# apache/yunikorn-k8shim

Measured on AMD Instinct MI355X. Metric: pod×node predicate evals/sec + decisions/sec, 50k nodes × 1M pods, higher is better.
Workload: dtype int64; 1 GPU; configs[2]: 50k nodes x 1M pods, NodeResourcesFit + TaintToleration + NodeAffinity; nodes_per_gpu=50000, total_nodes=50000, pods=1000000, templates=2000, pod_classes=2061, signature_planes=327, unique_requests=False, spread=False, gang_size=0, parallelism=single GPU

## Files before the change

yunikorn-k8shim_amd/csrc/engine/engine.hip:

```cpp
#include "../../../include/ykpred.h"

#include <hip/hip_runtime.h>
#include <dlfcn.h>
#include <rccl/rccl.h>

#include <algorithm>
#include <chrono>
#include <cstdio>
#include <cstdlib>
#include <cstring>
#include <mutex>
#include <string>
#include <unordered_map>
#include <vector>

#include "kernels.hip.h"

using ykk::i64;
using ykk::u64;

namespace {

thread_local std::string g_create_error;

// ... 259 lines not shown
  int rows_total = 0, rows_a = 0, row_capacity = 0;
  DevBuf d_pod_row;
  bool bands_enabled = true;
  int band_steps = 0;
  int band_steps_now = 128;
  int round_batched = -1;
  int round_node_assume = 1;
  int round_prof = 0;
  int fail_after = 0;
  int sig_wpl = 0;
  int combine_slices = 1;
  int decide_groups_from = 16384;
  int early_counts = 1;
  int max_lds_bytes = 64 * 1024;
  int num_cus = 256;
  int n_bands = 0, n_band_steps = 0, n_classes_a = 0, n_fix_rows = 0;
  std::vector<int32_t> h_class_slot_a;
  DevBuf d_band_tab, d_class_rows_a, d_class_list_a, d_class_slot_a, d_fix_row, d_fix_slot, d_chunk_zone;
  DevBuf d_class_list_b;
  int n_classes_b = 0;
  std::vector<int32_t> h_ch_zone;
  std::vector<uint8_t> h_row_stale;
  std::vector<int32_t> h_class_sig, h_class_pin, h_class_first, h_class_live;
  std::vector<std::vector<int32_t>> h_class_chunks;
  std::vector<int32_t> h_members, h_ch_class, h_ch_begin, h_ch_len, h_ch_first;
  int patch_chunks = 0;
  bool rank_valid = false;
  uint64_t specs_version = 1, ranked_specs_version = 0, ranked_nodes_epoch = 0;
  unsigned ranked_pre = 0, ranked_filt = 0;
  bool ranked_has_first = false;
  DevBuf d_round;
  DevBuf d_fx_off, d_fx_cls, d_fx_cnt, d_fx_occ, d_sp_sig_of;
  uint64_t fx_version = 0;
  bool fx_contrib = false, fx_ports = false;
  std::vector<int32_t> h_fx_off;
// ... 203 lines not shown
      long rows = 0;
      for (int c = 0; c < C; ++c)
        if (class_size[(size_t)c] >= need) rows += class_size[(size_t)c];
      return rows;
    };
    const long best = coverage(s_min);
    S = 128;
    while (S > s_min && (double)coverage(S) < 0.5 * (double)best) S /= 2;
  }
  while (S > 4 && (long)S * win / row_b >= (1L << 21)) S -= 4;
  e->band_steps_now = S;
  const int piece_min = piece_min_of(S);
  e->h_class_slot_a.assign((size_t)C, -1);
  e->h_pod_row.assign((size_t)P, -1);
  std::vector<ykk::BandEntry> band_tab;
  std::vector<int32_t> class_list_a, fix_row, fix_slot;
  int n_steps = 0, n_bands = 0, rows_a = 0;
  const bool geometry_ok = e->bands_enabled && e->N > 0 && (size_t)2 * KC * (size_t)row_b <= (size_t)std::min(ykk::kBandMaxLds, e->max_lds_bytes);
  if (geometry_ok) {
    long rows_needed = 0;
    for (int c = 0; c < C; ++c)
      if (class_size[(size_t)c] >= 2 * piece_min) {
        e->h_class_slot_a[(size_t)c] = (int32_t)class_list_a.size();
        class_list_a.push_back(c);
        rows_needed += class_size[(size_t)c];
      }
    if (rows_needed < (long)S * win / row_b / 4) {
      class_list_a.clear();
      std::fill(e->h_class_slot_a.begin(), e->h_class_slot_a.end(), -1);
    }
  }
// ... 87 lines not shown
      rows_a = (int)r_hi;
      if (band_steps_now < S) break;
    }
    if (ci < class_list_a.size()) ok = false;
    if (!ok) {
      class_list_a.clear();
      std::fill(e->h_class_slot_a.begin(), e->h_class_slot_a.end(), -1);
      std::fill(e->h_pod_row.begin(), e->h_pod_row.end(), -1);
      band_tab.clear();
      n_steps = n_bands = rows_a = 0;
    } else {
      n_bands = band;
      std::vector<int32_t> row_slot((size_t)rows_a, -1);
      for (int c : class_list_a)
        for (int i = class_off[(size_t)c]; i < class_off[(size_t)c + 1]; ++i) row_slot[(size_t)e->h_pod_row[(size_t)members[(size_t)i]]] = e->h_class_slot_a[(size_t)c];
      for (long s1 = 1; s1 <= n_steps; ++s1) {
        const long r = (s1 * win - 1) / row_b;
        if (r * row_b + row_b > s1 * win && r < rows_a && row_slot[(size_t)r] >= 0) {
          fix_row.push_back((int32_t)r);
          fix_slot.push_back(row_slot[(size_t)r]);
        }
      }
    }
  }
  int next_row = rows_a;
  e->h_class_sweep.assign((size_t)C, 0);
  e->sweep_ready = false;
  e->sweep_runs = 0;
  e->run_ranges = 0;
  e->walk2_chunks = -1;
  e->index_rows_needed = e->index_rows;
  for (int b = 0; b < ykk::kMaxIdxRows; ++b) e->sweep_rows[b] = 0;
  {
    std::vector<int32_t> order_b;
    for (int c = 0; c < C; ++c)
      if (e->h_class_slot_a[(size_t)c] < 0) order_b.push_back(c);
// ... 95 lines not shown
      if (kx != ky) return kx < ky;
      if (kx == 2) {
        if (cand_big[(size_t)x] != cand_big[(size_t)y]) return cand_big[(size_t)x] < cand_big[(size_t)y];
        if (cand_slot[(size_t)x] != cand_slot[(size_t)y]) return cand_slot[(size_t)x] < cand_slot[(size_t)y];
        if (cand_pos[(size_t)x] != cand_pos[(size_t)y]) return cand_pos[(size_t)x] < cand_pos[(size_t)y];
        return x < y;
      }
      if (key(x, 0) != key(y, 0)) return key(x, 0) < key(y, 0);
      return x < y;
    });
    std::vector<int32_t> first_row_of((size_t)C, -1);
    for (int32_t c : order_b) {
      first_row_of[(size_t)c] = next_row;
      for (int i = class_off[(size_t)c]; i < class_off[(size_t)c + 1]; ++i) e->h_pod_row[(size_t)members[(size_t)i]] = next_row++;
    }
    e->n_classes_b = (int)order_b.size();
    TRY(upload(e, e->d_class_list_b, order_b.data(), order_b.size(), st));
    std::vector<ykk::SweepRun> runs;
    e->run_classes = e->run_units = e->run_rows = 0;
    if (runs_possible) {
      std::vector<ykk::RunClass> rcs;
      std::vector<int32_t> starts;
      for (size_t i = 0; i < order_b.size();) {
        const int32_t c = order_b[i];
        if (kind_of(c) != 1) {
          ++i;
          continue;
        }
        size_t j = i;
        long rows_in_run = 0;
// ... 230 lines not shown
            if (sr >= 0)
              for (int k = 0; k < R1; ++k)
                if (e->h_res_rows[(size_t)sr * (size_t)R1 + (size_t)k] > 0 && (e->h_res_rows[(size_t)sr * (size_t)R1 + (size_t)k] >> ykk::kRowBigShift)) { ++t_single_big; break; }
          }
        }
        fprintf(stderr, "fused: %d classes, %d rows, %d combinations; chunk writers keep %ld classes / %ld rows of zone B (%ld single-row: %ld share their affinity signature, %ld with an index row, %ld spread, %ld pinned)\n",
                e->fuse_count, e->fuse_row_count, e->fuse_combos, t_cls, t_rows, t_single, t_single_shared, t_single_big, t_single_spread, t_pinned);
      }
    }
  }
  e->rows_total = next_row;
  e->rows_a = rows_a;
  e->n_bands = n_bands;
  e->n_band_steps = n_steps;
  e->n_classes_a = (int)class_list_a.size();
  e->n_fix_rows = (int)fix_row.size();
  if (e->row_capacity && e->rows_total > e->row_capacity)
    return fail(e, YKPRED_E_INVALID, "the bitmap needs more rows than ykpred_set_row_capacity allows");
  const int cm = e->chunk_members;
  struct Chunk {
    int32_t cls, begin, len, first, first_row;
  };
  std::vector<Chunk> chunks;
  for (int c = 0; c < C; ++c)
    for (int b = class_off[(size_t)c]; b < class_off[(size_t)c + 1]; b += cm)
      chunks.push_back({c, b, std::min(cm, class_off[(size_t)c + 1] - b), b == class_off[(size_t)c] ? 1 : 0, e->h_pod_row[(size_t)members[(size_t)b]]});
  if (e->chunk_sorted)
    std::stable_sort(chunks.begin(), chunks.end(), [](const Chunk& x, const Chunk& y) { return x.first_row < y.first_row; });
  auto &ch_class = e->h_ch_class, &ch_begin = e->h_ch_begin, &ch_len = e->h_ch_len, &ch_first = e->h_ch_first;
  ch_class.clear();
  ch_begin.clear();
// ... 27 lines not shown
  e->h_row_stale.assign((size_t)P, 0);
  e->C = C;
  e->NC = (int)ch_class.size();
  e->patch_chunks = 0;
  TRY(upload(e, e->d_pod_class, pod_class.data(), pod_class.size(), st));
  TRY(upload(e, e->d_class_sig, class_sig.data(), class_sig.size(), st));
  TRY(upload(e, e->d_class_pin, class_pin.data(), class_pin.size(), st));
  TRY(upload(e, e->d_class_first, e->h_class_first.data(), e->h_class_first.size(), st));
  TRY(upload(e, e->d_members, member_rows.data(), member_rows.size(), st));
  TRY(upload(e, e->d_pod_row, e->h_pod_row.data(), e->h_pod_row.size(), st));
  TRY(upload(e, e->d_chunk_zone, e->h_ch_zone.data(), e->h_ch_zone.size(), st));
  TRY(upload(e, e->d_chunk_list_b, chunk_list_b.data(), chunk_list_b.size(), st));
  TRY(upload(e, e->d_band_tab, band_tab.data(), band_tab.size(), st));
  TRY(upload(e, e->d_class_list_a, class_list_a.data(), class_list_a.size(), st));
  TRY(upload(e, e->d_class_slot_a, e->h_class_slot_a.data(), e->h_class_slot_a.size(), st));
  TRY(upload(e, e->d_fix_row, fix_row.data(), fix_row.size(), st));
  TRY(upload(e, e->d_fix_slot, fix_slot.data(), fix_slot.size(), st));
  HIPCHK(e->d_class_rows_a.ensure((size_t)std::max<size_t>(class_list_a.size(), 1) * (size_t)e->row_stride * sizeof(u64)));
  TRY(upload(e, e->d_chunk_class, ch_class.data(), ch_class.size(), st));
  TRY(upload(e, e->d_chunk_begin, ch_begin.data(), ch_begin.size(), st));
  TRY(upload(e, e->d_chunk_len, ch_len.data(), ch_len.size(), st));
  TRY(upload(e, e->d_chunk_first, ch_first.data(), ch_first.size(), st));
  HIPCHK(e->d_class_count.ensure((size_t)std::max(C, 1) * sizeof(int)));
  HIPCHK(e->d_class_best.ensure((size_t)std::max(C, 1) * sizeof(int)));
  HIPCHK(hipStreamSynchronize(st));
  e->classes_dirty = false;
  e->layout_version++;
  e->last_eval_valid = false;
  return YKPRED_OK;
}

int ensure_planes(ykpred_engine* e, hipStream_t st) {
  int rows = 0;
// ... 454 lines not shown
  if (e->comm) (void)rccl()->CommDestroy(e->comm);
  e->comm = nullptr;
  for (DevBuf* b : {&e->d_gathered, &e->d_gathered_map, &e->d_xkey, &e->d_xcand}) b->release();
  for (auto& g : e->graphs) (void)hipGraphExecDestroy(g.second);
  e->graphs.clear();
  for (DevBuf* b : {&e->d_alloc, &e->d_req, &e->d_allowed, &e->d_count, &e->d_nflags, &e->d_taints, &e->d_labels, &e->d_domain, &e->d_selcount, &e->d_ports, &e->d_sig_ports, &e->d_swanted,
                    &e->d_sp_cnt_prev, &e->d_sp_present_prev, &e->d_sp_min_prev, &e->d_sig_changed, &e->d_class_dirty,
                    &e->d_spec_spread, &e->d_sp_coff, &e->d_sp_c, &e->d_sp_aff, &e->d_sp_tol, &e->d_sp_cnt, &e->d_sp_present, &e->d_sp_min,
                    &e->planes_canon, &e->planes_ranked, &e->base_canon, &e->base_ranked, &e->d_rankbuf, &e->d_score, &e->d_key,
                    &e->d_rank, &e->d_perm, &e->d_sreq, &e->d_stol, &e->d_sflags, &e->d_aff_off, &e->d_aff_terms, &e->d_pre_off,
                    &e->d_pre_terms, &e->d_dim_val, &e->d_dim_order, &e->d_dim_chunk_dim, &e->d_dim_chunk_begin, &e->d_dim_chunk_len,
                    &e->d_res_rows, &e->d_big_dim, &e->d_walk_big, &e->d_walk_begin, &e->d_walk_len, &e->d_sfree_c, &e->d_pmask_c,
                    &e->d_sfree_r, &e->d_pmask_r, &e->d_rbits_c, &e->d_sorted, &e->d_sorted_off, &e->d_ent_c, &e->d_agree, &e->d_topo_agree, &e->d_bytes_gather, &e->d_fuse_rec, &e->d_fuse_combo_rec, &e->d_fuse_combo, &e->d_run_ranges, &e->d_no_decide, &e->d_glin_r, &e->d_run_classes, &e->d_run_units, &e->d_sweep_rows, &e->d_sweep_runs, &e->d_sweep_units, &e->d_chunk_list_b0, &e->d_walk2_order, &e->d_walk2_big, &e->d_walk2_begin, &e->d_walk2_len, &e->d_idx_c, &e->d_win_r, &e->d_pfx_r, &e->d_slice_desc, &e->d_slice_general, &e->d_chunk_list_b, &e->d_first_r, &e->d_sig_tol, &e->d_sig_tolflags, &e->d_sig_aff_flags, &e->d_sig_aff_off,
                    &e->d_sig_aff_terms, &e->d_sig_pre_off, &e->d_sig_pre_terms, &e->d_pod_spec, &e->d_pod_pin, &e->d_pod_class,
                    &e->d_class_sig, &e->d_class_pin, &e->d_class_first, &e->d_class_word, &e->d_chunk_class, &e->d_chunk_begin, &e->d_chunk_len, &e->d_chunk_first,
                    &e->d_pod_row, &e->d_band_tab, &e->d_class_rows_a, &e->d_class_list_a, &e->d_class_slot_a, &e->d_fix_row, &e->d_fix_slot, &e->d_chunk_zone,
                    &e->d_members, &e->d_patches, &e->d_rows, &e->d_row_count, &e->d_row_best, &e->d_class_count, &e->d_class_best, &e->d_bitmap, &e->d_counts, &e->d_decisions, &e->d_keys, &e->d_scratch,
                    &e->d_member_key, &e->d_name_rank, &e->d_member_tie, &e->d_class_rows_all, &e->d_gathered_classes, &e->d_class_rows_slot,
                    &e->d_class_sig_ident, &e->d_expand_count, &e->d_layout_hash, &e->d_gathered_pod_class, &e->d_row_pod,
                    &e->d_round, &e->d_fx_off, &e->d_fx_cls, &e->d_fx_cnt, &e->d_fx_occ, &e->d_sp_sig_of, &e->d_class_list_b, &e->d_gathered, &e->d_gathered_map,
                    &e->d_xkey, &e->d_xcand})
    b->release();
  if (e->ev_ready)
    for (auto& ev : e->ev) (void)hipEventDestroy(ev);
  if (e->ev_fork) (void)hipEventDestroy(e->ev_fork);
  if (e->ev_join) (void)hipEventDestroy(e->ev_join);
  if (e->ev_planes) (void)hipEventDestroy(e->ev_planes);
  if (e->ev_counts) (void)hipEventDestroy(e->ev_counts);
  if (e->ev_zero) (void)hipEventDestroy(e->ev_zero);
  if (e->h_round_pinned) (void)hipHostFree(e->h_round_pinned);
  if (e->ev_eval_done) (void)hipEventDestroy(e->ev_eval_done);
// ... 791 lines not shown
                         pr, n_decide, e->row_words, e->d_perm.as<int>(), e->d_rank.as<int>(), pin_on, e->d_class_best.as<int>(), n_decide <= 4096 ? 1 : 0);
    }
    tm.end(sb, "k_decide");
  }
  const bool skip_combine = a->options & YKPRED_EVAL_SKIP_BITMAP;
  const bool dirty_only = a->options & YKPRED_EVAL_DIRTY_CLASSES;
  const int* class_dirty = nullptr;
  if (!skip_combine && dirty_only) {
    HIPCHK(e->d_class_dirty.ensure((size_t)std::max(e->C, 1) * sizeof(int)));
    hipLaunchKernelGGL(ykk::k_mark_dirty_classes, dim3((unsigned)((e->C + ykk::kBlock - 1) / ykk::kBlock)), dim3(ykk::kBlock), 0, st, e->C,
                       e->d_class_sig.as<int>(), e->d_sig_changed.as<int>(), e->d_class_dirty.as<int>(), e->d_class_count.as<int>());
    class_dirty = e->d_class_dirty.as<int>();
  }
  const bool small_chunks = (long)e->NC * e->wave_combine_below > (long)P;
  const bool counts_early = e->early_counts != 0 && !skip_combine && !dirty_only && e->n_classes_a > 0 && e->patch_chunks == 0 && !small_chunks && e->n_classes_b <= 16384;
  bool scattered = false;
  if (!skip_combine && !dirty_only && !counts_early) {
    if (zero_counts_beside) HIPCHK(hipStreamWaitEvent(st, e->ev_zero, 0));
    else HIPCHK(hipMemsetAsync(e->d_class_count.p, 0, (size_t)e->C * sizeof(int), st));
  }
  if (!skip_combine) {
    int tpg = ykk::kBlock;
    while (tpg > ykk::kWave && (tpg / 2) * 2 >= e->row_stride) tpg /= 2;
    const int seg = tpg * ykk::kCombineUnroll * 2;
    const bool listed = !dirty_only && e->patch_chunks == 0;
    const bool short_list = use_sweep && (fuse_on || e->fuse_count == 0);
    const int* chunk_list = listed ? (short_list ? e->d_chunk_list_b0 : e->d_chunk_list_b).as<int>() : nullptr;
    const int n_run = listed ? (short_list ? e->NCB0 : e->NCB) : e->NC;
    dim3 grid((unsigned)std::max(n_run, 1), (unsigned)((e->row_stride + seg - 1) / seg));
    hipStream_t sz = st;
    if (!dirty_only && e->n_classes_a > 0) {
      tm.begin(st);
      const int n_counted_b = counts_early ? e->n_classes_b : 0;
      hipLaunchKernelGGL(ykk::k_class_rows, dim3((unsigned)((e->n_classes_a + n_counted_b + ykk::kWavesPerBlock - 1) / ykk::kWavesPerBlock)), dim3(ykk::kBlock), 0, st,
                         ct, pc, e->d_class_list_a.as<int>(), e->n_classes_a, e->row_words, e->row_stride, pin_on, e->d_class_rows_a.as<u64>(),
                         e->d_class_count.as<int>(), (const int*)nullptr, e->d_class_list_b.as<int>(), n_counted_b);
      tm.end(st, "k_class_rows");
      if (counts_early && want_dec) {
        HIPCHK(hipEventRecord(e->ev_counts, st));
        HIPCHK(hipStreamWaitEvent(sb, e->ev_counts, 0));
        tm.begin(sb);
        hipLaunchKernelGGL(ykk::k_scatter, dim3((unsigned)((P + ykk::kBlock - 1) / ykk::kBlock)), dim3(ykk::kBlock), 0, sb, P,
                           e->d_pod_class.as<int>(), e->d_class_count.as<int>(), e->d_class_best.as<int>(), e->d_key.as<u64>(),
                           want_cnt ? (int*)e->last_counts : nullptr, (int*)e->last_decisions, want_keys ? (i64*)e->last_keys : nullptr);
        tm.end(sb, "k_scatter");
        scattered = true;
      }
      const size_t lds_bytes = (size_t)2 * ykk::kBandClasses * (size_t)e->row_stride * sizeof(u64);
      if (lds_bytes > 64 * 1024)
        HIPCHK(hipFuncSetAttribute((const void*)ykk::k_expand_bands, hipFuncAttributeMaxDynamicSharedMemorySize, (int)lds_bytes));
      tm.begin(st);
      hipLaunchKernelGGL(ykk::k_expand_bands, dim3((unsigned)ykk::kBandGroups), dim3(ykk::kBandBlock), lds_bytes, st, bitmap,
                         e->d_class_rows_a.as<u64>(), e->d_band_tab.as<ykk::BandEntry>(), e->n_bands, e->row_stride);
      if (e->n_fix_rows > 0 && !counts_early)
        hipLaunchKernelGGL(ykk::k_fix_rows, dim3((unsigned)e->n_fix_rows), dim3(ykk::kBlock), 0, st, bitmap, e->d_class_rows_a.as<u64>(),
                           e->d_fix_row.as<int>(), e->d_fix_slot.as<int>(), e->n_fix_rows, e->row_stride);
      tm.end(st, "k_expand_bands");
    }
    if (use_sweep && e->run_classes > 0) {
      ykk::WalkStage rstage{};
      rstage.n = (int)e->h_stage_rows.size();
      for (int k = 0; k < rstage.n; ++k) rstage.row[k] = e->h_stage_rows[(size_t)k];
      const int its = (e->row_stride + ykk::kWave - 1) / ykk::kWave;
      int segs = (its + ykk::kWalkMaxIt - 1) / ykk::kWalkMaxIt, nit = (its + segs - 1) / segs;
      while (nit > 1 && ykk::runs_lds_bytes(rstage.n, nit) > (size_t)e->max_lds_bytes) {
        ++segs;
        nit = (its + segs - 1) / segs;
      }
      const int n_long = segs - (nit * segs - its);
      const size_t lds = ykk::runs_lds_bytes(rstage.n, nit);
      const int per_cu = lds * 2 <= (size_t)e->max_lds_bytes ? 2 : 1;
// ... 66 lines not shown
      auto launch_wide = [&](const ykk::FuseRec* recs, int n, u64* out, int* counts) {
        if (wpl == 5) launch_fused(ykk::k_fused_rows<5, 8>, recs, n, out, counts);
        else if (wpl == 2) launch_fused(ykk::k_fused_rows<2, 8>, recs, n, out, counts);
        else launch_fused(ykk::k_fused_rows<1, 8>, recs, n, out, counts);
      };
      if (e->fuse_combos > 0) {
        launch_wide(e->d_fuse_combo_rec.as<ykk::FuseRec>(), e->fuse_combos, e->d_fuse_combo.as<u64>(), nullptr);
        if (wpl == 5) launch_fused(ykk::k_fused_rows<5, 2>, e->d_fuse_rec.as<ykk::FuseRec>(), e->fuse_count, bitmap, e->d_class_count.as<int>());
        else if (wpl == 2) launch_fused(ykk::k_fused_rows<2, 2>, e->d_fuse_rec.as<ykk::FuseRec>(), e->fuse_count, bitmap, e->d_class_count.as<int>());
        else launch_fused(ykk::k_fused_rows<1, 2>, e->d_fuse_rec.as<ykk::FuseRec>(), e->fuse_count, bitmap, e->d_class_count.as<int>());
      } else {
        launch_wide(e->d_fuse_rec.as<ykk::FuseRec>(), e->fuse_count, bitmap, e->d_class_count.as<int>());
      }
      tm.end(sz, "k_fused_rows");
    }
    tm.begin(sz);
    int walk_nit = 0, walk_segs = 0, walk_long = 0;
    ykk::WalkStage wstage{};
    wstage.n = (int)e->h_stage_rows.size();
    for (int k = 0; k < wstage.n; ++k) wstage.row[k] = e->h_stage_rows[(size_t)k];
    bool slices = small_chunks && e->combine_slices != 0 && pc.n_big > 0 && pc.res != nullptr && !(use_sweep && e->sweep_min_run <= 1 && listed);
    if (slices) {
      const int its = (e->row_stride + ykk::kWave - 1) / ykk::kWave;
      const size_t lds_cap = std::min((size_t)e->max_lds_bytes, (size_t)80 * 1024);
      walk_segs = (its + ykk::kWalkMaxIt - 1) / ykk::kWalkMaxIt;
      walk_nit = (its + walk_segs - 1) / walk_segs;
      while (walk_nit > 1 && ykk::walk_lds_bytes(pc.n_big, wstage.n, walk_nit) > lds_cap) {
        ++walk_segs;
        walk_nit = (its + walk_segs - 1) / walk_segs;
      }
      walk_long = walk_segs - (walk_nit * walk_segs - its);
// ... 27 lines not shown
        }
        return fail(e, YKPRED_E_INVALID, "k_walk_rows: no kernel for " + std::to_string(nit) + " word groups per lane");
      };
      {
        const int n_short = walk_segs - walk_long, nit_last = n_short > 0 ? walk_nit - 1 : walk_nit;
        const int long_plain = n_short > 0 ? walk_long : walk_long - 1, short_plain = n_short > 0 ? n_short - 1 : 0;
        TRY(launch_segments(walk_nit, long_plain, 0, false));
        TRY(launch_segments(walk_nit - 1, short_plain, walk_long * walk_nit * ykk::kWave, false));
        TRY(launch_segments(nit_last, 1, (long_plain * walk_nit + short_plain * (walk_nit - 1)) * ykk::kWave, true));
      }
      tm.end(sz, "k_walk_rows");
      tm.begin(sz);
      hipLaunchKernelGGL(ykk::k_combine_wave, dim3((unsigned)((e->NC + ykk::kWavesPerBlock - 1) / ykk::kWavesPerBlock)), dim3(ykk::kBlock), 0, sz, ct,
                         pc, bitmap, e->row_words, e->row_stride, pin_on, e->d_class_count.as<int>(), e->NC, class_dirty,
                         e->d_slice_desc.as<ykk::SliceDesc>(), e->d_slice_general.as<int>(), (const int*)nullptr);
    } else if (counts_early) {
      const ykk::FixRows fix{e->d_class_rows_a.as<u64>(), e->d_fix_row.as<int>(), e->d_fix_slot.as<int>(), e->n_fix_rows};
      const int blocks = n_run + e->n_fix_rows;
      if (blocks > 0)
        hipLaunchKernelGGL(ykk::k_combine, dim3((unsigned)blocks, grid.y), dim3(ykk::kBlock), (size_t)e->combine_lds_bytes, sz, ct, pc, bitmap, e->row_words,
                           e->row_stride, pin_on, (int*)nullptr, tpg, class_dirty, chunk_list, fix, n_run);
    } else if (n_run == 0) {
    } else if (small_chunks) {
      const dim3 wgrid((unsigned)((std::max(n_run, 1) + ykk::kWavesPerBlock - 1) / ykk::kWavesPerBlock));
      hipLaunchKernelGGL(ykk::k_combine_wave, wgrid, dim3(ykk::kBlock), 0, sz, ct, pc, bitmap, e->row_words, e->row_stride, pin_on,
                         e->d_class_count.as<int>(), n_run, class_dirty, (const ykk::SliceDesc*)nullptr, (const int*)nullptr, chunk_list);
    } else {
      hipLaunchKernelGGL(ykk::k_combine, grid, dim3(ykk::kBlock), (size_t)e->combine_lds_bytes, sz, ct, pc, bitmap, e->row_words, e->row_stride,
                         pin_on, e->d_class_count.as<int>(), tpg, class_dirty, chunk_list, ykk::FixRows{nullptr, nullptr, nullptr, 0}, n_run);
    }
    tm.end(sz, dirty_only ? "k_combine(dirty classes)" : "k_combine");
  }
  if (want_dec) {
    HIPCHK(hipEventRecord(e->ev_join, sb));
    HIPCHK(hipStreamWaitEvent(st, e->ev_join, 0));
  }
  if ((want_dec || want_cnt) && !scattered) {
    tm.begin(st);
    hipLaunchKernelGGL(ykk::k_scatter, dim3((unsigned)((P + ykk::kBlock - 1) / ykk::kBlock)), dim3(ykk::kBlock), 0, st, P,
                       e->d_pod_class.as<int>(), e->d_class_count.as<int>(), e->d_class_best.as<int>(), e->d_key.as<u64>(),
                       want_cnt ? (int*)e->last_counts : nullptr, want_dec ? (int*)e->last_decisions : nullptr,
                       want_keys ? (i64*)e->last_keys : nullptr);
    tm.end(st, "k_scatter");
  }
  HIPCHK(hipGetLastError());
  return YKPRED_OK;
// ... 1761 lines not shown
    hipLaunchKernelGGL(ykk::k_identity_sigs, dim3((unsigned)((C + ykk::kBlock - 1) / ykk::kBlock)), dim3(ykk::kBlock), 0, st, C, e->d_class_sig_ident.as<int>());
    e->ident_classes = C;
  }
  HIPCHK(e->d_expand_count.ensure((size_t)C * sizeof(int)));
  ykk::ClassTable ct{e->d_class_sig_ident.as<int>(), e->d_class_pin.as<int>(), e->d_chunk_class.as<int>(), e->d_chunk_begin.as<int>(),
                     e->d_chunk_len.as<int>(), e->d_chunk_first.as<int>(), e->d_members.as<int>(), e->d_chunk_zone.as<int>(), 0, nullptr};
  ykk::Planes pl{nullptr, class_rows, nullptr, nullptr, e->row_stride, nullptr, 0, nullptr, 0, nullptr, 0, nullptr, 0, 0, 0, 0, 0, nullptr, nullptr, nullptr, nullptr, nullptr};
  if (e->n_classes_a > 0) {
    HIPCHK(e->d_class_rows_slot.ensure((size_t)e->n_classes_a * (size_t)e->row_stride * sizeof(u64)));
    hipLaunchKernelGGL(ykk::k_pick_class_rows, dim3((unsigned)e->n_classes_a), dim3(ykk::kBlock), 0, st, class_rows, e->d_class_list_a.as<int>(),
                       e->n_classes_a, e->row_stride, e->d_class_rows_slot.as<u64>());
    const size_t lds_bytes = (size_t)2 * ykk::kBandClasses * (size_t)e->row_stride * sizeof(u64);
    if (lds_bytes > 64 * 1024)
      HIPCHK(hipFuncSetAttribute((const void*)ykk::k_expand_bands, hipFuncAttributeMaxDynamicSharedMemorySize, (int)lds_bytes));
    hipLaunchKernelGGL(ykk::k_expand_bands, dim3((unsigned)ykk::kBandGroups), dim3(ykk::kBandBlock), lds_bytes, st, out, e->d_class_rows_slot.as<u64>(),
                       e->d_band_tab.as<ykk::BandEntry>(), e->n_bands, e->row_stride);
    if (e->n_fix_rows > 0)
      hipLaunchKernelGGL(ykk::k_fix_rows, dim3((unsigned)e->n_fix_rows), dim3(ykk::kBlock), 0, st, out, e->d_class_rows_slot.as<u64>(),
                         e->d_fix_row.as<int>(), e->d_fix_slot.as<int>(), e->n_fix_rows, e->row_stride);
  }
  if ((long)e->NC * e->wave_combine_below > (long)P) {
    hipLaunchKernelGGL(ykk::k_combine_wave, dim3((unsigned)((e->NC + ykk::kWavesPerBlock - 1) / ykk::kWavesPerBlock)), dim3(ykk::kBlock), 0, st, ct, pl,
                       out, e->row_stride, e->row_stride, 0, e->d_expand_count.as<int>(), e->NC, (const int*)nullptr, (const ykk::SliceDesc*)nullptr,
                       (const int*)nullptr, (const int*)nullptr);
  } else {
    int tpg = ykk::kBlock;
    while (tpg > ykk::kWave && (tpg / 2) * 2 >= e->row_stride) tpg /= 2;
    const int seg = tpg * ykk::kCombineUnroll * 2;
    dim3 grid((unsigned)e->NC, (unsigned)((e->row_stride + seg - 1) / seg));
    hipLaunchKernelGGL(ykk::k_combine, grid, dim3(ykk::kBlock), (size_t)e->combine_lds_bytes, st, ct, pl, out, e->row_stride, e->row_stride, 0,
                       e->d_expand_count.as<int>(), tpg, (const int*)nullptr, (const int*)nullptr, ykk::FixRows{nullptr, nullptr, nullptr, 0}, e->NC);
  }
  HIPCHK(hipGetLastError());
  return YKPRED_OK;
}
int expand_peer_rows_into(ykpred_engine_t* e, const u64* class_rows, const int* pod_class, u64* out, hipStream_t st) {
  if (e->P == 0) return YKPRED_OK;
  const int n_rows = std::max(std::max(e->rows_total, e->row_capacity), 1);
  if (e->row_pod_version != e->layout_version) {
    HIPCHK(e->d_row_pod.ensure((size_t)n_rows * sizeof(int)));
    HIPCHK(hipMemsetAsync(e->d_row_pod.p, 0xff, (size_t)n_rows * sizeof(int), st));
    hipLaunchKernelGGL(ykk::k_invert_row_map, dim3((unsigned)((e->P + ykk::kBlock - 1) / ykk::kBlock)), dim3(ykk::kBlock), 0, st, e->d_pod_row.as<int>(), e->P,
                       e->d_row_pod.as<int>());
    e->row_pod_version = e->layout_version;
  }
  const int row_groups = (n_rows + ykk::kExpandRows - 1) / ykk::kExpandRows;
// ... 178 lines not shown
```

yunikorn-k8shim_amd/csrc/engine/kernels.hip.h:

```cpp
#pragma once
#include <hip/hip_runtime.h>
#include <stdint.h>

#include <type_traits>

namespace ykk {

typedef unsigned long long u64;
typedef long long i64;

constexpr int kMaxR = 8;
constexpr int kMaxKT = 4;
constexpr int kMaxW = 8;
constexpr int kMaxWTotal = 32;
constexpr int kMaxKD = 8;
constexpr int kMaxKP = 4;

constexpr int kWave = 64;
constexpr int kBlock = 256;
constexpr int kWavesPerBlock = kBlock / kWave;
constexpr int kSigsPerBlock = 16;
constexpr int kSigsPerBlockMany = 64;
constexpr int kManySigs = 4096;
__host__ __device__ inline int sigs_per_block(int D) { return D > kManySigs ? kSigsPerBlockMany : kSigsPerBlock; }
// ... 1058 lines not shown
        pos = lo;
      }
      v &= cr.ipm[i][(size_t)w * 65 + min(pos, 64)];
    }
  return v;
}
__device__ __forceinline__ u64 class_word(const ClassRows& cr, int w) {
  u64 v = ~0ull;
#pragma unroll
  for (int i = 0; i < kMaxClassRows; ++i)
    if (i < cr.n) v &= cr.row[i][w];
  if (cr.ni) v &= class_idx_word(cr, w);
  return v;
}

struct FixRows {
  const u64* class_rows;
  const int* rows;
  const int* slots;
  int n;
};
__device__ __forceinline__ void fix_row(const FixRows& f, int i, u64* __restrict__ out, int row_stride) {
  typedef u64 u64x2 __attribute__((ext_vector_type(2)));
  if (i >= f.n) return;
  const u64* src = f.class_rows + (size_t)f.slots[i] * row_stride;
  u64* dst = out + (size_t)f.rows[i] * row_stride;
  for (int w = threadIdx.x * 2; w < row_stride; w += 2 * kBlock) *(u64x2*)(dst + w) = *(const u64x2*)(src + w);
}
__global__ __launch_bounds__(kBlock) void k_combine(ClassTable ct, Planes pl, u64* __restrict__ bitmap, int row_words, int row_stride,
                                                    int pin_enabled, int* __restrict__ class_count, int tpg,
                                                    const int* __restrict__ class_dirty ,
                                                    const int* __restrict__ chunk_list ,
                                                    FixRows fix ,
                                                    int n_run) {
  constexpr int WPL = 2;
  if ((int)blockIdx.x >= n_run) {
    if (blockIdx.y == 0) fix_row(fix, (int)blockIdx.x - n_run, bitmap, row_stride);
    return;
  }
  const bool all_fail = pin_enabled & 2;
  pin_enabled &= 1;
  const int chunk = chunk_list ? chunk_list[blockIdx.x] : (int)blockIdx.x;
  const int cls = ct.chunk_class[chunk];
  if (class_dirty ? !class_dirty[cls] : chunk_elsewhere(ct, chunk)) return;
  const int begin = ct.chunk_begin[chunk];
  const int len = ct.chunk_len[chunk];
  const int sr = ct.sig[cls * 4 + 0], st = ct.sig[cls * 4 + 1], sa = ct.sig[cls * 4 + 2], ss = ct.sig[cls * 4 + 3];
  const int pin = pin_enabled ? ct.pin[cls] : -1;
  const int lane = threadIdx.x % kWave;
  const int group = threadIdx.x / tpg, groups = kBlock / tpg, t = threadIdx.x % tpg;
  const int seg_base = blockIdx.y * (tpg * kCombineUnroll * WPL);
  const ClassRows cr = class_rows(pl, sr, st, sa, ss);

  u64 v[kCombineUnroll][WPL];
// ... 763 lines not shown
      if (__builtin_amdgcn_readfirstlane(db.x) != run) break;
    }
  }
}

constexpr int kBandGroups = 256;
constexpr int kBandClasses = 4;
constexpr int kBandMaxLds = 150 * 1024;
struct BandEntry {
  int slot[kBandClasses];
  int xb[kBandClasses - 1];
  int sb[kBandClasses - 1];
  int steps, first_step;
  int n, pad;
};

__global__ __launch_bounds__(kBlock) void k_class_rows(ClassTable ct, Planes pl, const int* __restrict__ class_list, int n_list, int row_words,
                                                       int row_stride, int pin_enabled, u64* __restrict__ row_table,
                                                       int* __restrict__ class_count, const int* __restrict__ class_dirty,
                                                       const int* __restrict__ class_list_b, int n_b) {
  typedef u64 u64x2 __attribute__((ext_vector_type(2)));
  const bool all_fail = pin_enabled & 2;
  pin_enabled &= 1;
  const int k = blockIdx.x * kWavesPerBlock + threadIdx.x / kWave;
  if (k >= n_list + n_b) return;
  const bool store = k < n_list;
  const int cls = store ? class_list[k] : class_list_b[k - n_list];
  if (class_dirty && !class_dirty[cls]) return;
  const int lane = threadIdx.x % kWave;
  const int sr = ct.sig[cls * 4 + 0], st = ct.sig[cls * 4 + 1], sa = ct.sig[cls * 4 + 2], ss = ct.sig[cls * 4 + 3];
  const int pin = pin_enabled ? ct.pin[cls] : -1;
  const ClassRows cr = class_rows(pl, sr, st, sa, ss);
  u64* dst = row_table + (size_t)k * row_stride;
  int pc = 0;
  for (int w = 2 * lane; w < row_stride; w += 2 * kWave) {
    u64x2 x = {0, 0};
    if (w < row_words && pin != -2 && !all_fail) {
      x = u64x2{~0ull, ~0ull};
#pragma unroll
      for (int i = 0; i < kMaxClassRows; ++i)
        if (i < cr.n) x &= *(const u64x2*)(cr.row[i] + w);
      if (cr.ni) {
// ... 4 lines not shown
      if (pin >= 0) {
        x.x &= (w == (pin >> 6)) ? (1ull << (pin & 63)) : 0ull;
        x.y &= (w + 1 == (pin >> 6)) ? (1ull << (pin & 63)) : 0ull;
      }
    }
    pc += __popcll(x.x) + __popcll(x.y);
    if (store) *(u64x2*)(dst + w) = x;
  }
#pragma unroll
  for (int off = 32; off > 0; off >>= 1) pc += __shfl_down(pc, off, kWave);
  if (lane == 0) class_count[cls] = pc;
}

constexpr int kBandBlock = kBlock + kWave;
__global__ __launch_bounds__(kBandBlock) void k_expand_bands(u64* __restrict__ out, const u64* __restrict__ class_rows,
                                                             const BandEntry* __restrict__ tab, int n_bands, int row_stride) {
  typedef u64 u64x2 __attribute__((ext_vector_type(2)));
  extern __shared__ u64 band_lds[];
  const int b = blockIdx.x, tid = threadIdx.x;
  const int row_b = row_stride * 8;
  constexpr long kWin = (long)kBandGroups * 4096;
  if (tid >= kBlock) {
    const int lane = tid - kBlock;
    const int pieces = row_stride / 2;
    auto load_rows = [&](int band) {
      const BandEntry be = tab[(size_t)band * kBandGroups + b];
#pragma unroll
      for (int c = 0; c < kBandClasses; ++c) {
        if (c >= be.n && c > 0) break;
        const u64x2* src = (const u64x2*)(class_rows + (size_t)be.slot[c] * row_stride);
        u64x2* dst = (u64x2*)(band_lds + (size_t)((band & 1) * kBandClasses + c) * row_stride);
        for (int i0 = 0; i0 < pieces; i0 += 4 * kWave) {
          u64x2 r[4];
#pragma unroll
          for (int k = 0; k < 4; ++k)
            if (i0 + k * kWave + lane < pieces) r[k] = src[i0 + k * kWave + lane];
#pragma unroll
          for (int k = 0; k < 4; ++k)
            if (i0 + k * kWave + lane < pieces) dst[i0 + k * kWave + lane] = r[k];
        }
      }
    };
    load_rows(0);
    __syncthreads();
    for (int band = 0; band < n_bands; ++band) {
      if (band + 1 < n_bands) load_rows(band + 1);
      __syncthreads();
    }
    return;
  }
  __syncthreads();
  const int p = b * 4096 + tid * 16;
  const unsigned urow_b = (unsigned)row_b;
  const unsigned dcol = (unsigned)(kWin % row_b);
  unsigned ucol = (unsigned)(p % row_b);
  for (int band = 0; band < n_bands; ++band) {
    const BandEntry cur = tab[(size_t)band * kBandGroups + b];
    const int s0 = cur.first_step, s1 = s0 + cur.steps;
    const char* lds = (const char*)(band_lds + (size_t)(band & 1) * kBandClasses * row_stride);
    unsigned kb[kBandClasses - 1];
#pragma unroll
// ... 24 lines not shown
          if (live[u]) *(u64x2*)(win_base + p) = v[u];
          win_base += kWin;
        }
      }
    };
    if (cur.n <= 1)
      run_band(std::integral_constant<int, 1>{});
    else if (cur.n == 2)
      run_band(std::integral_constant<int, 2>{});
    else if (cur.n == 3)
      run_band(std::integral_constant<int, 3>{});
    else
      run_band(std::integral_constant<int, kBandClasses>{});
    __syncthreads();
  }
}
__global__ __launch_bounds__(kBlock) void k_fix_rows(u64* __restrict__ out, const u64* __restrict__ class_rows, const int* __restrict__ rows,
                                                     const int* __restrict__ slots, int n, int row_stride) {
  typedef u64 u64x2 __attribute__((ext_vector_type(2)));
  if ((int)blockIdx.x >= n) return;
  const u64* src = class_rows + (size_t)slots[blockIdx.x] * row_stride;
  u64* dst = out + (size_t)rows[blockIdx.x] * row_stride;
  for (int w = threadIdx.x * 2; w < row_stride; w += 2 * kBlock) *(u64x2*)(dst + w) = *(const u64x2*)(src + w);
}

__global__ __launch_bounds__(kBlock) void k_decide(ClassTable ct, Planes ranked, int n_classes, int row_words, const int* __restrict__ perm,
                                                   const int* __restrict__ rank, int pin_enabled, int* __restrict__ class_best, int eager) {
  int cls = blockIdx.x * kWavesPerBlock + threadIdx.x / kWave;
  if (cls >= n_classes) return;
  if (ct.decide_list) cls = ct.decide_list[cls];
  const int lane = threadIdx.x % kWave;
  const int sr = ct.sig[cls * 4 + 0], st = ct.sig[cls * 4 + 1], sa = ct.sig[cls * 4 + 2], ss = ct.sig[cls * 4 + 3];
  const bool all_fail = pin_enabled & 2;
  const int pin = (pin_enabled & 1) ? ct.pin[cls] : -1;
  int best = -1;
  const ClassRows cr = class_rows(ranked, sr, st, sa, ss);
  if (pin == -2 || all_fail) {
    best = -1;
// ... 1940 lines not shown
```

Before: 42760 billion evals/s.

## Fold boundary-row fixups and B-class rows into band expansion kernel

Removes the separate k_fix_rows launch and the fix-row tail blocks in k_combine. The partial head of each band-boundary row is now copied inside k_expand_bands from the class row table. When the B-class rows fit within the band step count, k_class_rows also stores the B-class rows into the slot table. The band kernel's loader wave then copies them into the bitmap, letting the trailing k_combine launch be skipped. This costs extra row-table memory and puts more copy work on the band loader wave.

Result: slower. 42020 billion evals/s (-1.7%).

```diff
diff --git a/yunikorn-k8shim_amd/csrc/engine/engine.hip b/yunikorn-k8shim_amd/csrc/engine/engine.hip
--- a/yunikorn-k8shim_amd/csrc/engine/engine.hip
+++ b/yunikorn-k8shim_amd/csrc/engine/engine.hip
@@ -297,11 +297,12 @@
   int early_counts = 1;
   int max_lds_bytes = 64 * 1024;
   int num_cus = 256;
-  int n_bands = 0, n_band_steps = 0, n_classes_a = 0, n_fix_rows = 0;
+  int n_bands = 0, n_band_steps = 0, n_classes_a = 0;
   std::vector<int32_t> h_class_slot_a;
-  DevBuf d_band_tab, d_class_rows_a, d_class_list_a, d_class_slot_a, d_fix_row, d_fix_slot, d_chunk_zone;
+  DevBuf d_band_tab, d_class_rows_a, d_class_list_a, d_class_slot_a, d_head_slot, d_ride_slot, d_chunk_zone;
   DevBuf d_class_list_b;
   int n_classes_b = 0;
+  int n_ride_rows = 0, ride_rows_total = 0;
   std::vector<int32_t> h_ch_zone;
   std::vector<uint8_t> h_row_stale;
   std::vector<int32_t> h_class_sig, h_class_pin, h_class_first, h_class_live;
@@ -535,7 +536,7 @@
   e->h_class_slot_a.assign((size_t)C, -1);
   e->h_pod_row.assign((size_t)P, -1);
   std::vector<ykk::BandEntry> band_tab;
-  std::vector<int32_t> class_list_a, fix_row, fix_slot;
+  std::vector<int32_t> class_list_a, head_slot, ride_slot;
   int n_steps = 0, n_bands = 0, rows_a = 0;
   const bool geometry_ok = e->bands_enabled && e->N > 0 && (size_t)2 * KC * (size_t)row_b <= (size_t)std::min(ykk::kBandMaxLds, e->max_lds_bytes);
   if (geometry_ok) {
@@ -653,12 +654,10 @@
       std::vector<int32_t> row_slot((size_t)rows_a, -1);
       for (int c : class_list_a)
         for (int i = class_off[(size_t)c]; i < class_off[(size_t)c + 1]; ++i) row_slot[(size_t)e->h_pod_row[(size_t)members[(size_t)i]]] = e->h_class_slot_a[(size_t)c];
+      head_slot.assign((size_t)n_steps + 1, -1);
       for (long s1 = 1; s1 <= n_steps; ++s1) {
         const long r = (s1 * win - 1) / row_b;
-        if (r * row_b + row_b > s1 * win && r < rows_a && row_slot[(size_t)r] >= 0) {
-          fix_row.push_back((int32_t)r);
-          fix_slot.push_back(row_slot[(size_t)r]);
-        }
+        if (r * row_b + row_b > s1 * win && r < rows_a) head_slot[(size_t)s1] = row_slot[(size_t)r];
       }
     }
   }
@@ -784,6 +783,8 @@
       first_row_of[(size_t)c] = next_row;
       for (int i = class_off[(size_t)c]; i < class_off[(size_t)c + 1]; ++i) e->h_pod_row[(size_t)members[(size_t)i]] = next_row++;
     }
+    if (rows_a > 0 && next_row - rows_a <= n_steps)
+      for (size_t k = 0; k < order_b.size(); ++k) ride_slot.insert(ride_slot.end(), (size_t)class_size[(size_t)order_b[k]], (int32_t)(class_list_a.size() + k));
     e->n_classes_b = (int)order_b.size();
     TRY(upload(e, e->d_class_list_b, order_b.data(), order_b.size(), st));
     std::vector<ykk::SweepRun> runs;
@@ -1044,7 +1045,8 @@
   e->n_bands = n_bands;
   e->n_band_steps = n_steps;
   e->n_classes_a = (int)class_list_a.size();
-  e->n_fix_rows = (int)fix_row.size();
+  e->n_ride_rows = (int)ride_slot.size();
+  e->ride_rows_total = next_row;
   if (e->row_capacity && e->rows_total > e->row_capacity)
     return fail(e, YKPRED_E_INVALID, "the bitmap needs more rows than ykpred_set_row_capacity allows");
   const int cm = e->chunk_members;
@@ -1102,9 +1104,9 @@
   TRY(upload(e, e->d_band_tab, band_tab.data(), band_tab.size(), st));
   TRY(upload(e, e->d_class_list_a, class_list_a.data(), class_list_a.size(), st));
   TRY(upload(e, e->d_class_slot_a, e->h_class_slot_a.data(), e->h_class_slot_a.size(), st));
-  TRY(upload(e, e->d_fix_row, fix_row.data(), fix_row.size(), st));
-  TRY(upload(e, e->d_fix_slot, fix_slot.data(), fix_slot.size(), st));
-  HIPCHK(e->d_class_rows_a.ensure((size_t)std::max<size_t>(class_list_a.size(), 1) * (size_t)e->row_stride * sizeof(u64)));
+  TRY(upload(e, e->d_head_slot, head_slot.data(), head_slot.size(), st));
+  TRY(upload(e, e->d_ride_slot, ride_slot.data(), ride_slot.size(), st));
+  HIPCHK(e->d_class_rows_a.ensure((size_t)std::max<size_t>(class_list_a.size() + (ride_slot.empty() ? 0 : (size_t)e->n_classes_b), 1) * (size_t)e->row_stride * sizeof(u64)));
   TRY(upload(e, e->d_chunk_class, ch_class.data(), ch_class.size(), st));
   TRY(upload(e, e->d_chunk_begin, ch_begin.data(), ch_begin.size(), st));
   TRY(upload(e, e->d_chunk_len, ch_len.data(), ch_len.size(), st));
@@ -1589,7 +1591,7 @@
                     &e->d_sfree_r, &e->d_pmask_r, &e->d_rbits_c, &e->d_sorted, &e->d_sorted_off, &e->d_ent_c, &e->d_agree, &e->d_topo_agree, &e->d_bytes_gather, &e->d_fuse_rec, &e->d_fuse_combo_rec, &e->d_fuse_combo, &e->d_run_ranges, &e->d_no_decide, &e->d_glin_r, &e->d_run_classes, &e->d_run_units, &e->d_sweep_rows, &e->d_sweep_runs, &e->d_sweep_units, &e->d_chunk_list_b0, &e->d_walk2_order, &e->d_walk2_big, &e->d_walk2_begin, &e->d_walk2_len, &e->d_idx_c, &e->d_win_r, &e->d_pfx_r, &e->d_slice_desc, &e->d_slice_general, &e->d_chunk_list_b, &e->d_first_r, &e->d_sig_tol, &e->d_sig_tolflags, &e->d_sig_aff_flags, &e->d_sig_aff_off,
                     &e->d_sig_aff_terms, &e->d_sig_pre_off, &e->d_sig_pre_terms, &e->d_pod_spec, &e->d_pod_pin, &e->d_pod_class,
                     &e->d_class_sig, &e->d_class_pin, &e->d_class_first, &e->d_class_word, &e->d_chunk_class, &e->d_chunk_begin, &e->d_chunk_len, &e->d_chunk_first,
-                    &e->d_pod_row, &e->d_band_tab, &e->d_class_rows_a, &e->d_class_list_a, &e->d_class_slot_a, &e->d_fix_row, &e->d_fix_slot, &e->d_chunk_zone,
+                    &e->d_pod_row, &e->d_band_tab, &e->d_class_rows_a, &e->d_class_list_a, &e->d_class_slot_a, &e->d_head_slot, &e->d_ride_slot, &e->d_chunk_zone,
                     &e->d_members, &e->d_patches, &e->d_rows, &e->d_row_count, &e->d_row_best, &e->d_class_count, &e->d_class_best, &e->d_bitmap, &e->d_counts, &e->d_decisions, &e->d_keys, &e->d_scratch,
                     &e->d_member_key, &e->d_name_rank, &e->d_member_tie, &e->d_class_rows_all, &e->d_gathered_classes, &e->d_class_rows_slot,
                     &e->d_class_sig_ident, &e->d_expand_count, &e->d_layout_hash, &e->d_gathered_pod_class, &e->d_row_pod,
@@ -2411,6 +2413,7 @@
   }
   const bool small_chunks = (long)e->NC * e->wave_combine_below > (long)P;
   const bool counts_early = e->early_counts != 0 && !skip_combine && !dirty_only && e->n_classes_a > 0 && e->patch_chunks == 0 && !small_chunks && e->n_classes_b <= 16384;
+  const bool ride = counts_early && e->n_ride_rows > 0 && e->rows_total == e->ride_rows_total;
   bool scattered = false;
   if (!skip_combine && !dirty_only && !counts_early) {
     if (zero_counts_beside) HIPCHK(hipStreamWaitEvent(st, e->ev_zero, 0));
@@ -2431,7 +2434,7 @@
       const int n_counted_b = counts_early ? e->n_classes_b : 0;
       hipLaunchKernelGGL(ykk::k_class_rows, dim3((unsigned)((e->n_classes_a + n_counted_b + ykk::kWavesPerBlock - 1) / ykk::kWavesPerBlock)), dim3(ykk::kBlock), 0, st,
                          ct, pc, e->d_class_list_a.as<int>(), e->n_classes_a, e->row_words, e->row_stride, pin_on, e->d_class_rows_a.as<u64>(),
-                         e->d_class_count.as<int>(), (const int*)nullptr, e->d_class_list_b.as<int>(), n_counted_b);
+                         e->d_class_count.as<int>(), (const int*)nullptr, e->d_class_list_b.as<int>(), n_counted_b, ride ? 1 : 0);
       tm.end(st, "k_class_rows");
       if (counts_early && want_dec) {
         HIPCHK(hipEventRecord(e->ev_counts, st));
@@ -2448,10 +2451,8 @@
         HIPCHK(hipFuncSetAttribute((const void*)ykk::k_expand_bands, hipFuncAttributeMaxDynamicSharedMemorySize, (int)lds_bytes));
       tm.begin(st);
       hipLaunchKernelGGL(ykk::k_expand_bands, dim3((unsigned)ykk::kBandGroups), dim3(ykk::kBandBlock), lds_bytes, st, bitmap,
-                         e->d_class_rows_a.as<u64>(), e->d_band_tab.as<ykk::BandEntry>(), e->n_bands, e->row_stride);
-      if (e->n_fix_rows > 0 && !counts_early)
-        hipLaunchKernelGGL(ykk::k_fix_rows, dim3((unsigned)e->n_fix_rows), dim3(ykk::kBlock), 0, st, bitmap, e->d_class_rows_a.as<u64>(),
-                           e->d_fix_row.as<int>(), e->d_fix_slot.as<int>(), e->n_fix_rows, e->row_stride);
+                         e->d_class_rows_a.as<u64>(), e->d_band_tab.as<ykk::BandEntry>(), e->n_bands, e->row_stride,
+                         ykk::BandRide{e->d_head_slot.as<int>(), e->d_ride_slot.as<int>(), ride ? e->n_ride_rows : 0, e->rows_a});
       tm.end(st, "k_expand_bands");
     }
     if (use_sweep && e->run_classes > 0) {
@@ -2548,7 +2549,8 @@
       }
       tm.end(sz, "k_fused_rows");
     }
-    tm.begin(sz);
+    const bool tail = !(ride || (counts_early && n_run == 0));
+    if (tail) tm.begin(sz);
     int walk_nit = 0, walk_segs = 0, walk_long = 0;
     ykk::WalkStage wstage{};
     wstage.n = (int)e->h_stage_rows.size();
@@ -2606,12 +2608,11 @@
       hipLaunchKernelGGL(ykk::k_combine_wave, dim3((unsigned)((e->NC + ykk::kWavesPerBlock - 1) / ykk::kWavesPerBlock)), dim3(ykk::kBlock), 0, sz, ct,
                          pc, bitmap, e->row_words, e->row_stride, pin_on, e->d_class_count.as<int>(), e->NC, class_dirty,
                          e->d_slice_desc.as<ykk::SliceDesc>(), e->d_slice_general.as<int>(), (const int*)nullptr);
+    } else if (ride) {
     } else if (counts_early) {
-      const ykk::FixRows fix{e->d_class_rows_a.as<u64>(), e->d_fix_row.as<int>(), e->d_fix_slot.as<int>(), e->n_fix_rows};
-      const int blocks = n_run + e->n_fix_rows;
-      if (blocks > 0)
-        hipLaunchKernelGGL(ykk::k_combine, dim3((unsigned)blocks, grid.y), dim3(ykk::kBlock), (size_t)e->combine_lds_bytes, sz, ct, pc, bitmap, e->row_words,
-                           e->row_stride, pin_on, (int*)nullptr, tpg, class_dirty, chunk_list, fix, n_run);
+      if (n_run > 0)
+        hipLaunchKernelGGL(ykk::k_combine, grid, dim3(ykk::kBlock), (size_t)e->combine_lds_bytes, sz, ct, pc, bitmap, e->row_words, e->row_stride, pin_on,
+                           (int*)nullptr, tpg, class_dirty, chunk_list, n_run);
     } else if (n_run == 0) {
     } else if (small_chunks) {
       const dim3 wgrid((unsigned)((std::max(n_run, 1) + ykk::kWavesPerBlock - 1) / ykk::kWavesPerBlock));
@@ -2619,9 +2620,9 @@
                          e->d_class_count.as<int>(), n_run, class_dirty, (const ykk::SliceDesc*)nullptr, (const int*)nullptr, chunk_list);
     } else {
       hipLaunchKernelGGL(ykk::k_combine, grid, dim3(ykk::kBlock), (size_t)e->combine_lds_bytes, sz, ct, pc, bitmap, e->row_words, e->row_stride,
-                         pin_on, e->d_class_count.as<int>(), tpg, class_dirty, chunk_list, ykk::FixRows{nullptr, nullptr, nullptr, 0}, n_run);
-    }
-    tm.end(sz, dirty_only ? "k_combine(dirty classes)" : "k_combine");
+                         pin_on, e->d_class_count.as<int>(), tpg, class_dirty, chunk_list, n_run);
+    }
+    if (tail) tm.end(sz, dirty_only ? "k_combine(dirty classes)" : "k_combine");
   }
   if (want_dec) {
     HIPCHK(hipEventRecord(e->ev_join, sb));
@@ -4413,10 +4414,7 @@
     if (lds_bytes > 64 * 1024)
       HIPCHK(hipFuncSetAttribute((const void*)ykk::k_expand_bands, hipFuncAttributeMaxDynamicSharedMemorySize, (int)lds_bytes));
     hipLaunchKernelGGL(ykk::k_expand_bands, dim3((unsigned)ykk::kBandGroups), dim3(ykk::kBandBlock), lds_bytes, st, out, e->d_class_rows_slot.as<u64>(),
-                       e->d_band_tab.as<ykk::BandEntry>(), e->n_bands, e->row_stride);
-    if (e->n_fix_rows > 0)
-      hipLaunchKernelGGL(ykk::k_fix_rows, dim3((unsigned)e->n_fix_rows), dim3(ykk::kBlock), 0, st, out, e->d_class_rows_slot.as<u64>(),
-                         e->d_fix_row.as<int>(), e->d_fix_slot.as<int>(), e->n_fix_rows, e->row_stride);
+                       e->d_band_tab.as<ykk::BandEntry>(), e->n_bands, e->row_stride, ykk::BandRide{e->d_head_slot.as<int>(), nullptr, 0, e->rows_a});
   }
   if ((long)e->NC * e->wave_combine_below > (long)P) {
     hipLaunchKernelGGL(ykk::k_combine_wave, dim3((unsigned)((e->NC + ykk::kWavesPerBlock - 1) / ykk::kWavesPerBlock)), dim3(ykk::kBlock), 0, st, ct, pl,
@@ -4428,7 +4426,7 @@
     const int seg = tpg * ykk::kCombineUnroll * 2;
     dim3 grid((unsigned)e->NC, (unsigned)((e->row_stride + seg - 1) / seg));
     hipLaunchKernelGGL(ykk::k_combine, grid, dim3(ykk::kBlock), (size_t)e->combine_lds_bytes, st, ct, pl, out, e->row_stride, e->row_stride, 0,
-                       e->d_expand_count.as<int>(), tpg, (const int*)nullptr, (const int*)nullptr, ykk::FixRows{nullptr, nullptr, nullptr, 0}, e->NC);
+                       e->d_expand_count.as<int>(), tpg, (const int*)nullptr, (const int*)nullptr, e->NC);
   }
   HIPCHK(hipGetLastError());
   return YKPRED_OK;
diff --git a/yunikorn-k8shim_amd/csrc/engine/kernels.hip.h b/yunikorn-k8shim_amd/csrc/engine/kernels.hip.h
--- a/yunikorn-k8shim_amd/csrc/engine/kernels.hip.h
+++ b/yunikorn-k8shim_amd/csrc/engine/kernels.hip.h
@@ -1096,30 +1096,13 @@
   return v;
 }
 
-struct FixRows {
-  const u64* class_rows;
-  const int* rows;
-  const int* slots;
-  int n;
-};
-__device__ __forceinline__ void fix_row(const FixRows& f, int i, u64* __restrict__ out, int row_stride) {
-  typedef u64 u64x2 __attribute__((ext_vector_type(2)));
-  if (i >= f.n) return;
-  const u64* src = f.class_rows + (size_t)f.slots[i] * row_stride;
-  u64* dst = out + (size_t)f.rows[i] * row_stride;
-  for (int w = threadIdx.x * 2; w < row_stride; w += 2 * kBlock) *(u64x2*)(dst + w) = *(const u64x2*)(src + w);
-}
 __global__ __launch_bounds__(kBlock) void k_combine(ClassTable ct, Planes pl, u64* __restrict__ bitmap, int row_words, int row_stride,
                                                     int pin_enabled, int* __restrict__ class_count, int tpg,
                                                     const int* __restrict__ class_dirty ,
                                                     const int* __restrict__ chunk_list ,
-                                                    FixRows fix ,
                                                     int n_run) {
   constexpr int WPL = 2;
-  if ((int)blockIdx.x >= n_run) {
-    if (blockIdx.y == 0) fix_row(fix, (int)blockIdx.x - n_run, bitmap, row_stride);
-    return;
-  }
+  if ((int)blockIdx.x >= n_run) return;
   const bool all_fail = pin_enabled & 2;
   pin_enabled &= 1;
   const int chunk = chunk_list ? chunk_list[blockIdx.x] : (int)blockIdx.x;
@@ -1913,18 +1896,24 @@
   int steps, first_step;
   int n, pad;
 };
+struct BandRide {
+  const int* head_slot;
+  const int* ride_slot;
+  int n_ride, first_row;
+};
+constexpr int kBandPiece = 1024;
 
 __global__ __launch_bounds__(kBlock) void k_class_rows(ClassTable ct, Planes pl, const int* __restrict__ class_list, int n_list, int row_words,
                                                        int row_stride, int pin_enabled, u64* __restrict__ row_table,
                                                        int* __restrict__ class_count, const int* __restrict__ class_dirty,
-                                                       const int* __restrict__ class_list_b, int n_b) {
+                                                       const int* __restrict__ class_list_b, int n_b, int store_b) {
   typedef u64 u64x2 __attribute__((ext_vector_type(2)));
   const bool all_fail = pin_enabled & 2;
   pin_enabled &= 1;
   const int k = blockIdx.x * kWavesPerBlock + threadIdx.x / kWave;
   if (k >= n_list + n_b) return;
-  const bool store = k < n_list;
-  const int cls = store ? class_list[k] : class_list_b[k - n_list];
+  const bool store = k < n_list || store_b;
+  const int cls = k < n_list ? class_list[k] : class_list_b[k - n_list];
   if (class_dirty && !class_dirty[cls]) return;
   const int lane = threadIdx.x % kWave;
   const int sr = ct.sig[cls * 4 + 0], st = ct.sig[cls * 4 + 1], sa = ct.sig[cls * 4 + 2], ss = ct.sig[cls * 4 + 3];
@@ -1959,7 +1948,7 @@
 
 constexpr int kBandBlock = kBlock + kWave;
 __global__ __launch_bounds__(kBandBlock) void k_expand_bands(u64* __restrict__ out, const u64* __restrict__ class_rows,
-                                                             const BandEntry* __restrict__ tab, int n_bands, int row_stride) {
+                                                             const BandEntry* __restrict__ tab, int n_bands, int row_stride, BandRide ride) {
   typedef u64 u64x2 __attribute__((ext_vector_type(2)));
   extern __shared__ u64 band_lds[];
   const int b = blockIdx.x, tid = threadIdx.x;
@@ -1986,10 +1975,46 @@
         }
       }
     };
+    auto copy_pieces = [&](int first, int stride, int n, auto where) {
+      for (int q0 = first; q0 < n; q0 += 4 * stride) {
+        u64x2 r[4];
+        char* d[4];
+        bool on[4];
+#pragma unroll
+        for (int k = 0; k < 4; ++k) {
+          const int q = q0 + k * stride;
+          const char* src = nullptr;
+          d[k] = nullptr;
+          on[k] = q < n && lane * 16 < where(q, src, d[k]);
+          if (on[k]) r[k] = *(const u64x2*)(src + lane * 16);
+        }
+#pragma unroll
+        for (int k = 0; k < 4; ++k)
+          if (on[k]) *(u64x2*)(d[k] + lane * 16) = r[k];
+      }
+    };
+    const int row_pieces = (row_b + kBandPiece - 1) / kBandPiece;
+    const char* table = (const char*)class_rows;
     load_rows(0);
     __syncthreads();
     for (int band = 0; band < n_bands; ++band) {
       if (band + 1 < n_bands) load_rows(band + 1);
+      const BandEntry cur = tab[(size_t)band * kBandGroups + b];
+      copy_pieces(b, kBandGroups, cur.steps * row_pieces, [&](int q, const char*& src, char*& dst) {
+        const int s = cur.first_step + 1 + q / row_pieces, at = q % row_pieces * kBandPiece;
+        const int slot = ride.head_slot[s];
+        const long edge = (long)s * kWin;
+        const int h = (int)((row_b - edge % row_b) % row_b);
+        src = table + (size_t)(slot < 0 ? 0 : slot) * row_b + (row_b - h) + at;
+        dst = (char*)out + edge + at;
+        return slot < 0 ? 0 : h - at;
+      });
+      copy_pieces(band * kBandGroups + b, n_bands * kBandGroups, ride.n_ride * row_pieces, [&](int q, const char*& src, char*& dst) {
+        const int i = q / row_pieces, at = q % row_pieces * kBandPiece;
+        src = table + (size_t)ride.ride_slot[i] * row_b + at;
+        dst = (char*)out + (size_t)(ride.first_row + i) * row_b + at;
+        return row_b - at;
+      });
       __syncthreads();
     }
     return;
@@ -2044,14 +2069,6 @@
       run_band(std::integral_constant<int, kBandClasses>{});
     __syncthreads();
   }
-}
-__global__ __launch_bounds__(kBlock) void k_fix_rows(u64* __restrict__ out, const u64* __restrict__ class_rows, const int* __restrict__ rows,
-                                                     const int* __restrict__ slots, int n, int row_stride) {
-  typedef u64 u64x2 __attribute__((ext_vector_type(2)));
-  if ((int)blockIdx.x >= n) return;
-  const u64* src = class_rows + (size_t)slots[blockIdx.x] * row_stride;
-  u64* dst = out + (size_t)rows[blockIdx.x] * row_stride;
-  for (int w = threadIdx.x * 2; w < row_stride; w += 2 * kBlock) *(u64x2*)(dst + w) = *(const u64x2*)(src + w);
 }
 
 __global__ __launch_bounds__(kBlock) void k_decide(ClassTable ct, Planes ranked, int n_classes, int row_words, const int* __restrict__ perm,
```
